# diffqc/dqc

Hardware: AMD Instinct MI355X
Metric: SCF iterations/sec (Fock build + XC grid) per GPU, cc-pVDZ 20-atom (higher is better)
Workload: dtype f64

## Files before the change

dqc_amd/csrc/grid_density.hip:

```cpp
#include "grid_common.hpp"

namespace dqc {

constexpr int DEN_BM = 64;
constexpr int DEN_NT = DEN_BM * 4;
constexpr int DEN_KC = 16;
constexpr int DEN_SA = DEN_KC + 2;

#ifdef DEN_TRACE
__device__ long long g_den_trace[4 * 16384];
DQC_DEV void den_trace(int k) {
    if (threadIdx.x == 0 && blockIdx.x < 16384) {
        if (k == 0) {
            unsigned hw, xcc;
            asm volatile("s_getreg_b32 %0, hwreg(HW_REG_HW_ID)" : "=s"(hw));
            asm volatile("s_getreg_b32 %0, hwreg(HW_REG_XCC_ID)" : "=s"(xcc));
            g_den_trace[4 * blockIdx.x + 3] = (long long)(((xcc & 7u) << 8) | ((hw >> 8) & 0xffu));
        }
        g_den_trace[4 * blockIdx.x + k] = wall_clock64();
    }
}
#define DEN_TRACE_POINT(k) den_trace(k)
#else
#define DEN_TRACE_POINT(k)
#endif

#ifdef DEN_EXP_UNPAIRED
constexpr bool DEN_PAIRED = false;
#else
constexpr bool DEN_PAIRED = true;
#endif

constexpr int lr_panel_stride(int nct) {
    return (DEN_PAIRED && nct >= 2) ? nct * 16 + 1 : (((nct * 16) & 31) == 16 ? nct * 16 : nct * 16 + 16);
}

template <int NCT, bool GGA, int Q0 = 0>
DQC_DEV void rowdot_epilogue(const v4d (&acc)[NCT], double (&p)[4][GGA ? 4 : 1], const double *__restrict__ blk0,
                             const double *__restrict__ blkg, size_t cs, const int (&roff)[4], int col0) {
    constexpr int NQ = (GGA ? 4 : 1) - Q0, NB = 4 * NQ;
    if (NB == 0) return;
    constexpr int DP = 2;
    double t[DP][NCT];
    auto issue = [&](int bt, double (&dst)[NCT]) {
        const int r = bt / NQ, q = bt % NQ + Q0;
        const double *base = (q == 0 ? blk0 : blkg + q * cs) + col0;
#pragma unroll
        for (int ct = 0; ct < NCT; ct++) dst[ct] = base[roff[r] + ct * 16];
    };
#pragma unroll
    for (int b0 = 0; b0 < DP - 1 && b0 < NB; b0++) issue(b0, t[b0]);
#pragma unroll
    for (int bt = 0; bt < NB; bt++) {
        if (bt + DP - 1 < NB) issue(bt + DP - 1, t[(bt + DP - 1) % DP]);
        const int r = bt / NQ, q = bt % NQ + Q0;
#pragma unroll
        for (int ct = 0; ct < NCT; ct++) p[r][q] += acc[ct][r] * t[bt % DP][ct];
        __builtin_amdgcn_sched_barrier(0);
    }
}

template <int NCT, bool GGA, int Q0 = 0, int DP = 2>
DQC_DEV void rowdot_epilogue_paired(const v4d (&acc)[NCT], double (&p)[4][GGA ? 4 : 1], const double *__restrict__ blk0,
                                    const double *__restrict__ blkg, size_t cs, const int (&roff)[4], int lr, int col0) {
    constexpr int NQ = (GGA ? 4 : 1) - Q0, NB = 4 * NQ, NP = NCT / 2, ODD = NCT & 1;
    if (NB == 0) return;
    double2 t2[DP][NP > 0 ? NP : 1];
    double t1[DP];
    auto issue = [&](int bt, double2 (&d2)[NP > 0 ? NP : 1], double &d1) {
        const int r = bt / NQ, q = bt % NQ + Q0;
        const double *base = (q == 0 ? blk0 : blkg + q * cs) + col0;
#pragma unroll
        for (int m = 0; m < NP; m++) d2[m] = *reinterpret_cast<const double2 *>(base + roff[r] + m * 32);
        if (ODD) d1 = base[(roff[r] - lr) + (NCT - 1) * 16];
    };
#pragma unroll
    for (int b0 = 0; b0 < DP - 1 && b0 < NB; b0++) issue(b0, t2[b0], t1[b0]);
#pragma unroll
    for (int bt = 0; bt < NB; bt++) {
        if (bt + DP - 1 < NB) issue(bt + DP - 1, t2[(bt + DP - 1) % DP], t1[(bt + DP - 1) % DP]);
        const int r = bt / NQ, q = bt % NQ + Q0;
#pragma unroll
        for (int m = 0; m < NP; m++) p[r][q] += acc[2 * m][r] * t2[bt % DP][m].x + acc[2 * m + 1][r] * t2[bt % DP][m].y;
        if (ODD) p[r][q] += acc[NCT - 1][r] * t1[bt % DP];
        __builtin_amdgcn_sched_barrier(0);
    }
}

template <int NCT>
DQC_DEV void rowdot_epilogue_paired2(const v4d (&acc)[2][NCT], double (&p)[2][4][4], const double *__restrict__ blkg, size_t cs,
                                     const int (&roff)[4], int lr, int col0) {
    constexpr int NQ = 3, NB = 4 * NQ, NP = NCT / 2, ODD = NCT & 1, DP = 2;
    double2 t2[DP][NP > 0 ? NP : 1];
    double t1[DP];
    auto issue = [&](int bt, double2 (&d2)[NP > 0 ? NP : 1], double &d1) {
        const int r = bt / NQ, q = bt % NQ + 1;
        const double *base = blkg + q * cs + col0;
#pragma unroll
        for (int m = 0; m < NP; m++) d2[m] = *reinterpret_cast<const double2 *>(base + roff[r] + m * 32);
        if (ODD) d1 = base[(roff[r] - lr) + (NCT - 1) * 16];
    };
    issue(0, t2[0], t1[0]);
#pragma unroll
    for (int bt = 0; bt < NB; bt++) {
        if (bt + 1 < NB) issue(bt + 1, t2[(bt + 1) % DP], t1[(bt + 1) % DP]);
        const int r = bt / NQ, q = bt % NQ + 1;
#pragma unroll
        for (int sp = 0; sp < 2; sp++) {
#pragma unroll
            for (int m = 0; m < NP; m++) p[sp][r][q] += acc[sp][2 * m][r] * t2[bt % DP][m].x + acc[sp][2 * m + 1][r] * t2[bt % DP][m].y;
            if (ODD) p[sp][r][q] += acc[sp][NCT - 1][r] * t1[bt % DP];
        }
        __builtin_amdgcn_sched_barrier(0);
    }
}

template <int NCT, bool GGA>
__global__ __launch_bounds__(256, 2) void density_kernel(double *__restrict__ rho, double *__restrict__ grho,
                                                         const double *__restrict__ ao, int ngrid, int ld,
                                                         const double *__restrict__ dm, int ntile,
                                                         const double *__restrict__ aoe, int lda) {
    extern __shared__ __attribute__((aligned(16))) double lds[];
    constexpr int LSB = NCT * 16;
    constexpr int LSBP = lr_panel_stride(NCT);
    constexpr int A_SZ = DEN_BM * DEN_SA, B_SZ = DEN_KC * LSBP;
    constexpr int NB2 = (DEN_KC * LSB / 2 + DEN_NT - 1) / DEN_NT;
    constexpr int NKK = DEN_KC / 4;
    double *sA = lds, *sB = lds + 2 * A_SZ;
    const int tid = threadIdx.x, wave = tid >> 6, lane = tid & 63;
    const int lr = lane & 15, lk = lane >> 4;
    const int g0 = blockIdx.x * DEN_BM;
    const size_t cs = (size_t)ngrid * lda;
    const double *aoblk = ao + (size_t)g0 * lda;
    const double *aoeblk = aoe + (size_t)g0 * lda;
    const int rmax = ngrid - 1 - g0;
    const int arow = tid >> 2, aseg = (tid & 3) * 4;
    const int aoff = min(arow, rmax) * lda + aseg;

    double p[4][GGA ? 4 : 1];
#pragma unroll
    for (int r = 0; r < 4; r++)
#pragma unroll
        for (int q = 0; q < (GGA ? 4 : 1); q++) p[r][q] = 0.0;
    int roff[4];
#pragma unroll
    for (int r = 0; r < 4; r++) roff[r] = min(wave * 16 + lk + 4 * r, rmax) * lda + (DEN_PAIRED ? 2 : 1) * lr;

    DEN_TRACE_POINT(0);
    const int nk = ld / DEN_KC;
    for (int jnew = 0; jnew < ntile; jnew += NCT) {
        const int jc = min(jnew, ntile - NCT);
        v4d acc[NCT];
#pragma unroll
        for (int ct = 0; ct < NCT; ct++) acc[ct] = v4d{0, 0, 0, 0};
        double2 paA0 = make_double2(0.0, 0.0), paA1 = paA0, paB0 = paA0, paB1 = paA0, pbA[NB2], pbB[NB2];
        int boff[NB2];
        bool bzero[NB2];
#pragma unroll
        for (int i = 0; i < NB2; i++) {
            const int e = min((tid + i * DEN_NT) * 2, DEN_KC * LSB - 2);
            const int row = e / LSB, col = e - row * LSB;
            boff[i] = row * ld + jc * 16 + col;
            bzero[i] = jc * 16 + col < jnew * 16;
            pbA[i] = pbB[i] = make_double2(0.0, 0.0);
        }
#define DQC_DEN_PREF(KC, S, PART)                                                                          \
    {                                                                                                      \
        const int kq_ = min((KC), nk - 1);      \
        if ((PART) == 0) {                                                                                 \
            const double *s_ = aoblk + kq_ * DEN_KC + aoff;                                                \
            pa##S##0 = *reinterpret_cast<const double2 *>(s_);                                             \
            pa##S##1 = *reinterpret_cast<const double2 *>(s_ + 2);                                         \
        }                                                                                                  \
        const double *d_ = dm + (size_t)kq_ * DEN_KC * ld;                                                 \
        _Pragma("unroll") for (int i = 0; i < NB2; i++) {                                                  \
            if (i % NKK != (PART)) continue;                                                               \
            pb##S[i] = *reinterpret_cast<const double2 *>(d_ + boff[i]);                                   \
            if (bzero[i]) pb##S[i] = make_double2(0.0, 0.0);                                               \
        }                                                                                                  \
    }
#define DQC_DEN_STAGE(KC, S)                                                                               \
    if ((KC) < nk) {                                                                                       \
        const int buf_ = (KC) & 1;                                                                         \
        double *a_ = sA + buf_ * A_SZ + arow * DEN_SA + aseg;                                              \
        *reinterpret_cast<double2 *>(a_) = pa##S##0;                                                       \
        *reinterpret_cast<double2 *>(a_ + 2) = pa##S##1;                                                   \
        _Pragma("unroll") for (int i = 0; i < NB2; i++) {                                                  \
            const int e = (tid + i * DEN_NT) * 2;                                                          \
            const int row = e / LSB, col = e - row * LSB;                                                  \
            if (row < DEN_KC) {                                     \
                double *d = sB + buf_ * B_SZ + row * LSBP + col;                                           \
                d[0] = pb##S[i].x;                                                                         \
                d[1] = pb##S[i].y;                                                                         \
            }                                                                                              \
        }                                                                                                  \
    }
#define DQC_DEN_MFMAS(KC, S)                                                                               \
    {                                                                                                      \
        const int buf_ = (KC) & 1;                                                                         \
        const double *a = sA + buf_ * A_SZ + (wave * 16 + lr) * DEN_SA + lk;                               \
        const double *b = sB + buf_ * B_SZ + lk * LSBP + lr;                                               \
        const double *b2 = b + lr;  \
        _Pragma("unroll") for (int kk = 0; kk < NKK; kk++) {                                               \
            DQC_DEN_PREF((KC) + 2, S, kk)                     \
            const double av = a[kk * 4];                                                                   \
            _Pragma("unroll") for (int ct = 0; ct < NCT; ct++) {                                           \
                const double bv = (DEN_PAIRED && ct < 2 * (NCT / 2)) ? b2[kk * 4 * LSBP + 32 * (ct >> 1) + (ct & 1)] \
                                                                    : b[kk * 4 * LSBP + ct * 16];          \
                acc[ct] = mfma_f64(av, bv, acc[ct]);                                                       \
            }                                                                                              \
        }                                                                                                  \
    }
        __syncthreads();
#pragma unroll
        for (int part = 0; part < NKK; part++) DQC_DEN_PREF(0, A, part)
#pragma unroll
        for (int part = 0; part < NKK; part++) DQC_DEN_PREF(1, B, part)
        DQC_DEN_STAGE(0, A)
        __syncthreads();
        int kc = 0;
        for (; kc + 1 < nk; kc += 2) {
            DQC_DEN_MFMAS(kc, A)
            DQC_DEN_STAGE(kc + 1, B)
            __syncthreads();
            DQC_DEN_MFMAS(kc + 1, B)
            DQC_DEN_STAGE(kc + 2, A)
            __syncthreads();
        }
        if (kc < nk) {
            DQC_DEN_MFMAS(kc, A)
            __syncthreads();
        }
#undef DQC_DEN_PREF
#undef DQC_DEN_STAGE
#undef DQC_DEN_MFMAS
        DEN_TRACE_POINT(1);
#ifdef ABL_DEN_NO_EPI
        if (ngrid < 0)
#endif
        {
            if constexpr (DEN_PAIRED) rowdot_epilogue_paired<NCT, GGA>(acc, p, GGA ? aoblk : aoeblk, aoblk, cs, roff, lr, jc * 16);
            else rowdot_epilogue<NCT, GGA>(acc, p, GGA ? aoblk : aoeblk, aoblk, cs, roff, jc * 16);
        }
    }
#pragma unroll
    for (int r = 0; r < 4; r++)
#pragma unroll
        for (int q = 0; q < (GGA ? 4 : 1); q++) {
            double v = p[r][q];
            v += __shfl_xor(v, 1);
            v += __shfl_xor(v, 2);
            v += __shfl_xor(v, 4);
            v += __shfl_xor(v, 8);
            p[r][q] = v;
        }
    DEN_TRACE_POINT(2);
    if (lr == 0) {
#pragma unroll
        for (int r = 0; r < 4; r++) {
            const int row = g0 + wave * 16 + lk + 4 * r;
            if (row < ngrid) {
                rho[row] = p[r][0];
                if (GGA) {
                    grho[row] = 2.0 * p[r][1];
                    grho[(size_t)ngrid + row] = 2.0 * p[r][2];
                    grho[2 * (size_t)ngrid + row] = 2.0 * p[r][3];
                }
            }
        }
    }
}

template <int NCT>
static constexpr size_t density_lds_bytes() {
    constexpr int LSBP = lr_panel_stride(NCT);
    return sizeof(double) * 2 * (DEN_BM * DEN_SA + DEN_KC * LSBP);
}

template <bool GGA>
static int launch_density(int nct, dim3 grid, hipStream_t st, double *rho, double *grho, const double *ao,
                          int ngrid, int ld, const double *dm, int ntile, const double *aoe, int lda) {

#define DQC_DENS_CASE(N)                                                                                           \
    case N:                                                                                                        \
        if constexpr (!GGA || N <= 14) {           \
            (void)hipFuncSetAttribute((const void *)density_kernel<N, GGA>, hipFuncAttributeMaxDynamicSharedMemorySize, \
                                      (int)density_lds_bytes<N>());                                                \
            hipLaunchKernelGGL((density_kernel<N, GGA>), grid, dim3(DEN_NT), density_lds_bytes<N>(), st, rho, grho, ao, \
                               ngrid, ld, dm, ntile, aoe, lda);                                                     \
            return 0;                                                                                              \
        }                                                                                                          \
        break;
    switch (nct) {
        DQC_DENS_CASE(1) DQC_DENS_CASE(2) DQC_DENS_CASE(3) DQC_DENS_CASE(4) DQC_DENS_CASE(5) DQC_DENS_CASE(6)
        DQC_DENS_CASE(7) DQC_DENS_CASE(8) DQC_DENS_CASE(9) DQC_DENS_CASE(10) DQC_DENS_CASE(11) DQC_DENS_CASE(12)
        DQC_DENS_CASE(13) DQC_DENS_CASE(14) DQC_DENS_CASE(15) DQC_DENS_CASE(16)
    default:
        break;
    }
#undef DQC_DENS_CASE
    set_error("density: internal tile-count dispatch error");
    return DQC_EINVAL;
}


template <int NRT>
struct LrGeom {
    static constexpr int RP = NRT * 16;
    static constexpr int RPS = (RP & 31) == 16 ? RP : RP + 16;
};

template <int NRT, int NCT, bool GGA, int NS = 1>
__global__ __launch_bounds__(256, 2) void density_lr_kernel(double *__restrict__ rho, double *__restrict__ grho,
                                                            const double *__restrict__ ao, int ngrid, int ld,
                                                            const double *__restrict__ orb,
                                                            const double *__restrict__ orbt, int ntile, int lda) {
    extern __shared__ __attribute__((aligned(16))) double lds[];
    constexpr int RP = LrGeom<NRT>::RP, RPS = LrGeom<NRT>::RPS;
    constexpr int LSB = NCT * 16;
    constexpr int LSBP = lr_panel_stride(NCT);
    constexpr int A_SZ = DEN_BM * DEN_SA;
    constexpr int B_SZ = DEN_KC * (LSBP > RPS ? LSBP : RPS);
    constexpr int NL2 = (DEN_KC * RP / 2 + DEN_NT - 1) / DEN_NT;
    constexpr int NB2 = (DEN_KC * LSB / 2 + DEN_NT - 1) / DEN_NT;
    double *sA = lds, *sB = lds + 2 * A_SZ;
    const int tid = threadIdx.x, wave = tid >> 6, lane = tid & 63;
    const int lr = lane & 15, lk = lane >> 4;
    const int g0 = blockIdx.x * DEN_BM;
    const size_t cs = (size_t)ngrid * lda;
    const double *aoblk = ao + (size_t)g0 * lda;
    const int rmax = ngrid - 1 - g0;
    const int arow = tid >> 2, aseg = (tid & 3) * 4;
    const int aoff = min(arow, rmax) * lda + aseg;

    DEN_TRACE_POINT(0);
    v4d a1[NRT];
#pragma unroll
    for (int ct = 0; ct < NRT; ct++) a1[ct] = v4d{0, 0, 0, 0};
    {
        static_assert(NL2 <= 4, "L chunk wider than 4 double2 per thread");
        double2 pa0a, pa0b, pa1a, pa1b, pl0a, pl0b, pl0c, pl0d, pl1a, pl1b, pl1c, pl1d;
        pl0a = pl0b = pl0c = pl0d = pl1a = pl1b = pl1c = pl1d = make_double2(0.0, 0.0);
        const int nk = ld / DEN_KC;
        const int lo0 = min((tid + 0 * DEN_NT) * 2, DEN_KC * RP - 2), lo1 = min((tid + 1 * DEN_NT) * 2, DEN_KC * RP - 2);
        const int lo2 = min((tid + 2 * DEN_NT) * 2, DEN_KC * RP - 2), lo3 = min((tid + 3 * DEN_NT) * 2, DEN_KC * RP - 2);
#define DQC_LR_PREFETCH(KC, S)                                                                            \
    {                                                                                                     \
        const int kq = min((KC), nk - 1);      \
        const double *s_ = aoblk + kq * DEN_KC + aoff;                                                    \
        pa##S##a = *reinterpret_cast<const double2 *>(s_);                                                \
        pa##S##b = *reinterpret_cast<const double2 *>(s_ + 2);                                            \
        const double *l_ = orb + (size_t)kq * DEN_KC * RP;  \
        pl##S##a = *reinterpret_cast<const double2 *>(l_ + lo0);                                          \
        if (NL2 > 1) pl##S##b = *reinterpret_cast<const double2 *>(l_ + lo1);                             \
        if (NL2 > 2) pl##S##c = *reinterpret_cast<const double2 *>(l_ + lo2);                             \
        if (NL2 > 3) pl##S##d = *reinterpret_cast<const double2 *>(l_ + lo3);                             \
    }
#define DQC_LR_PUT(I, V)                                                                                  \
    {                                                                                                     \
        const int e_ = (tid + (I) * DEN_NT) * 2;                                                          \
        const int row_ = e_ / RP, col_ = e_ - row_ * RP;                                                  \
        if (row_ < DEN_KC) *reinterpret_cast<double2 *>(sB + buf_ * B_SZ + row_ * RPS + col_) = V;        \
    }
#define DQC_LR_STAGE(KC, S)                                                                               \
    if ((KC) < nk) {                                                                                      \
        const int buf_ = (KC) & 1;                                                                        \
        double *a_ = sA + buf_ * A_SZ + arow * DEN_SA + aseg;                                             \
        *reinterpret_cast<double2 *>(a_) = pa##S##a;                                                      \
        *reinterpret_cast<double2 *>(a_ + 2) = pa##S##b;                                                  \
        DQC_LR_PUT(0, pl##S##a)                                                                           \
        if (NL2 > 1) DQC_LR_PUT(1, pl##S##b)                                                              \
        if (NL2 > 2) DQC_LR_PUT(2, pl##S##c)                                                              \
        if (NL2 > 3) DQC_LR_PUT(3, pl##S##d)                                                              \
    }
#define DQC_LR_MFMAS(KC)                                                                                  \
    {                                                                                                     \
        const int buf_ = (KC) & 1;                                                                        \
        const double *b_ = sA + buf_ * A_SZ + (wave * 16 + lr) * DEN_SA + lk;  \
        const double *a_ = sB + buf_ * B_SZ + lk * RPS + lr;                   \
        _Pragma("unroll") for (int kk = 0; kk < DEN_KC / 4; kk++) {                                       \
            const double bv = b_[kk * 4];                                                                 \
            _Pragma("unroll") for (int ct = 0; ct < NRT; ct++)                                            \
                a1[ct] = mfma_f64(a_[kk * 4 * RPS + ct * 16], bv, a1[ct]);                                \
        }                                                                                                 \
    }
        DQC_LR_PREFETCH(0, 0)
        DQC_LR_PREFETCH(1, 1)
        DQC_LR_STAGE(0, 0)
        __syncthreads();
        int kc = 0;
        for (; kc + 1 < nk; kc += 2) {
            DQC_LR_PREFETCH(kc + 2, 0)
            DQC_LR_MFMAS(kc)
            DQC_LR_STAGE(kc + 1, 1)
            __syncthreads();
            DQC_LR_PREFETCH(kc + 3, 1)
            DQC_LR_MFMAS(kc + 1)
            DQC_LR_STAGE(kc + 2, 0)
            __syncthreads();
        }
        if (kc < nk) {
            DQC_LR_MFMAS(kc)
            __syncthreads();
        }
#undef DQC_LR_PREFETCH
#undef DQC_LR_STAGE
#undef DQC_LR_PUT
#undef DQC_LR_MFMAS
    }

    static_assert(NS == 1 || (NS == 2 && NRT % 2 == 0), "two spin channels of equal padded width");
    constexpr int NRU = NRT / NS;
#pragma unroll
    for (int sp = 0; sp < NS; sp++) {
        double rs = 0.0;
#pragma unroll
        for (int ct = sp * NRU; ct < (sp + 1) * NRU; ct++)
#pragma unroll
            for (int q = 0; q < 4; q++) rs += a1[ct][q] * a1[ct][q];
        rs += __shfl_xor(rs, 16);
        rs += __shfl_xor(rs, 32);
        const int row = g0 + wave * 16 + lr;
        if (lk == 0 && row < ngrid) rho[(size_t)sp * ngrid + row] = rs;
    }
    if (!GGA) return;

    double p[NS][4][GGA ? 4 : 1];
#pragma unroll
    for (int sp = 0; sp < NS; sp++)
#pragma unroll
    for (int r = 0; r < 4; r++)
#pragma unroll
        for (int q = 0; q < (GGA ? 4 : 1); q++) p[sp][r][q] = 0.0;
    int roff[4];
#pragma unroll
    for (int r = 0; r < 4; r++) roff[r] = min(wave * 16 + lk + 4 * r, rmax) * lda + (DEN_PAIRED ? 2 : 1) * lr;

    for (int jnew = 0; jnew < ntile; jnew += NCT) {
        const int jc = min(jnew, ntile - NCT);
        v4d acc[NS][NCT];
#pragma unroll
        for (int sp = 0; sp < NS; sp++)
#pragma unroll
        for (int ct = 0; ct < NCT; ct++) acc[sp][ct] = v4d{0, 0, 0, 0};
        double2 pb[NB2];
        int boff[NB2];
        bool bzero[NB2];
#pragma unroll
        for (int i = 0; i < NB2; i++) {
            const int e = min((tid + i * DEN_NT) * 2, DEN_KC * LSB - 2);
            const int row = e / LSB, col = e - row * LSB;
            boff[i] = row * ld + jc * 16 + col;
            bzero[i] = jc * 16 + col < jnew * 16;
        }
        auto prefetch = [&](int kc) {
            const double *l = orbt + (size_t)kc * DEN_KC * ld;
#pragma unroll
            for (int i = 0; i < NB2; i++) {
                pb[i] = *reinterpret_cast<const double2 *>(l + boff[i]);
                if (bzero[i]) pb[i] = make_double2(0.0, 0.0);
            }
        };
        auto stage = [&](int buf) {
#pragma unroll
            for (int i = 0; i < NB2; i++) {
                const int e = (tid + i * DEN_NT) * 2;
                const int row = e / LSB, col = e - row * LSB;
                if (row < DEN_KC) {
                    double *d = sB + buf * B_SZ + row * LSBP + col;
                    d[0] = pb[i].x;
                    d[1] = pb[i].y;
                }
            }
        };
        __syncthreads();
        prefetch(0);
        stage(0);
        __syncthreads();
#pragma unroll 1
        for (int kc = 0; kc < NRT; kc++) {
            const int buf = kc & 1;
            if (kc + 1 < NRT) prefetch(kc + 1);
            v4d a4 = a1[0];
#pragma unroll
            for (int c = 1; c < NRT; c++)
                if (kc == c) a4 = a1[c];
            const double *b = sB + buf * B_SZ + lk * LSBP + lr;
            const double *b2 = b + lr;
#pragma unroll
            for (int kk = 0; kk < 4; kk++) {
                const double av = a4[kk];
#pragma unroll
                for (int ct = 0; ct < NCT; ct++) {
                    const double bv = (DEN_PAIRED && ct < 2 * (NCT / 2)) ? b2[kk * 4 * LSBP + 32 * (ct >> 1) + (ct & 1)]
                                                                        : b[kk * 4 * LSBP + ct * 16];
                    if (NS == 1 || kc < NRU) acc[0][ct] = mfma_f64(av, bv, acc[0][ct]);
                    else acc[NS - 1][ct] = mfma_f64(av, bv, acc[NS - 1][ct]);
                }
            }
            if (kc + 1 < NRT) stage(buf ^ 1);
            __syncthreads();
        }
        DEN_TRACE_POINT(1);
        if constexpr (NS == 2) {
            static_assert(NS == 1 || (DEN_PAIRED && GGA), "spin-fused form: paired epilogue only");
            rowdot_epilogue_paired2<NCT>(acc, p, aoblk, cs, roff, lr, jc * 16);
        } else if constexpr (!DEN_PAIRED) rowdot_epilogue<NCT, GGA, 1>(acc[0], p[0], aoblk, aoblk, cs, roff, jc * 16);
        else if constexpr (GGA) rowdot_epilogue_paired<NCT, true, 1>(acc[0], p[0], aoblk, aoblk, cs, roff, lr, jc * 16);
        DEN_TRACE_POINT(2);
    }
#pragma unroll
    for (int sp = 0; sp < NS; sp++)
#pragma unroll
    for (int r = 0; r < 4; r++)
#pragma unroll
        for (int q = 0; q < (GGA ? 4 : 1); q++) {
            double v = p[sp][r][q];
            v += __shfl_xor(v, 1);
            v += __shfl_xor(v, 2);
            v += __shfl_xor(v, 4);
            v += __shfl_xor(v, 8);
            p[sp][r][q] = v;
        }
    if (lr == 0) {
#pragma unroll
        for (int sp = 0; sp < NS; sp++)
#pragma unroll
        for (int r = 0; r < 4; r++) {
            const int row = g0 + wave * 16 + lk + 4 * r;
            if (row < ngrid) {
                double *gs = grho + (size_t)sp * 3 * ngrid;
                gs[row] = 2.0 * p[sp][r][1];
                gs[(size_t)ngrid + row] = 2.0 * p[sp][r][2];
                gs[2 * (size_t)ngrid + row] = 2.0 * p[sp][r][3];
            }
        }
    }
}

template <int NRT, int NCT>
static constexpr size_t density_lr_lds_bytes() {
    constexpr int LSBP = lr_panel_stride(NCT);
    constexpr int RPS = LrGeom<NRT>::RPS;
    return sizeof(double) * 2 * (DEN_BM * DEN_SA + DEN_KC * (LSBP > RPS ? LSBP : RPS));
}

constexpr int lr_max_nct(int nrt) { return nrt <= 3 ? 14 : (nrt <= 4 ? 12 : 10); }

template <int NRT, bool GGA>
static int launch_density_lr_n(int nct, dim3 grid, hipStream_t st, double *rho, double *grho, const double *ao, int ngrid,
                               int ld, const double *orb, const double *orbt, int ntile, int lda) {
#define DQC_DLR_CASE(N)                                                                                          \
    case N:                                                                                                      \
        if constexpr (!GGA || N <= lr_max_nct(NRT)) {          \
            constexpr size_t shm = density_lr_lds_bytes<NRT, N>();                                               \
            auto kern = density_lr_kernel<NRT, N, GGA>;                                                          \
            (void)hipFuncSetAttribute((const void *)kern, hipFuncAttributeMaxDynamicSharedMemorySize, (int)shm); \
            hipLaunchKernelGGL(kern, grid, dim3(DEN_NT), shm, st, rho, grho, ao, ngrid, ld, orb, orbt, ntile, lda); \
            return 0;                                                                                            \
        }                                                                                                        \
        break;
    switch (nct) {
        DQC_DLR_CASE(1) DQC_DLR_CASE(2) DQC_DLR_CASE(3) DQC_DLR_CASE(4) DQC_DLR_CASE(5) DQC_DLR_CASE(6) DQC_DLR_CASE(7)
        DQC_DLR_CASE(8) DQC_DLR_CASE(9) DQC_DLR_CASE(10) DQC_DLR_CASE(11) DQC_DLR_CASE(12) DQC_DLR_CASE(13) DQC_DLR_CASE(14)
        DQC_DLR_CASE(15) DQC_DLR_CASE(16)
    default:
        break;
    }
#undef DQC_DLR_CASE
    set_error("density_lr: internal tile-count dispatch error");
    return DQC_EINVAL;
}

constexpr int ROLE_NT = 512;
constexpr unsigned ROLE_SPIN_CAP = 1u << 22;
constexpr int ROLE_DP = 3;

template <int NRT, int NT>
struct RoleGeom {
    static constexpr int RP = NRT * 16;
    static constexpr int S = NT * 16 + 1;
    static constexpr int P0 = (NT + 1) / 2;
    static constexpr int P1 = NT - P0;
    static constexpr int LT_SZ = (RP * S + 1) & ~1;
    static constexpr int MB_W = P0 * 256;
    static constexpr int SA_W = 2 * 16 * DEN_SA;
    static constexpr size_t lds_bytes() { return sizeof(double) * (LT_SZ + 4 * MB_W + 4 * SA_W) + 64; }
};

template <int NT>
DQC_DEV int role_col(int ct, int lr) {
    return ct < 2 * (NT / 2) ? 32 * (ct >> 1) + 2 * lr + (ct & 1) : ct * 16 + lr;
}

DQC_DEV void role_wait(unsigned *flag, unsigned want, unsigned *broken) {
    unsigned n = 0;
    while (__hip_atomic_load(flag, __ATOMIC_ACQUIRE, __HIP_MEMORY_SCOPE_WORKGROUP) < want) {
        if (__hip_atomic_load(broken, __ATOMIC_RELAXED, __HIP_MEMORY_SCOPE_WORKGROUP) != 0u) break;
        if (++n > ROLE_SPIN_CAP) {
            __hip_atomic_store(broken, 1u, __ATOMIC_RELAXED, __HIP_MEMORY_SCOPE_WORKGROUP);
            break;
        }
        __builtin_amdgcn_s_sleep(2);
    }
}

DQC_DEV void role_signal(unsigned *flag, unsigned v) {
    __hip_atomic_store(flag, v, __ATOMIC_RELEASE, __HIP_MEMORY_SCOPE_WORKGROUP);
}

template <int NRT, int NT>
__global__ __launch_bounds__(ROLE_NT, 1) void density_roles_kernel(double *__restrict__ rho, double *__restrict__ grho,
                                                                   const double *__restrict__ ao, int ngrid,
                                                                   const double *__restrict__ orbt, int lda) {
    using G = RoleGeom<NRT, NT>;
    constexpr int RP = G::RP, S = G::S, P0 = G::P0, P1 = G::P1, LD = NT * 16;
    constexpr int NPF = 4;
    static_assert(NT >= 2 && NT <= 14 && P1 >= 1, "one epilogue panel of 2..14 tiles");
    extern __shared__ __attribute__((aligned(16))) double lds[];
    double *sLT = lds, *sMB = lds + G::LT_SZ, *sAall = sMB + 4 * G::MB_W;
    unsigned *flags = reinterpret_cast<unsigned *>(sAall + 4 * G::SA_W);
    const int tid = threadIdx.x, lane = tid & 63;
    const int wave = __builtin_amdgcn_readfirstlane(tid >> 6);
    const int lr = lane & 15, lk = lane >> 4;
    const int ntiles = (ngrid + DEN_BM - 1) / DEN_BM;
    const size_t cs = (size_t)ngrid * lda;

    for (int e = tid; e < RP * LD; e += ROLE_NT) {
        const int r = e / LD, c = e - r * LD;
        sLT[r * S + c] = orbt[e];
    }
    if (tid < 16) flags[tid] = 0u;
    __syncthreads();
    const int w = wave & 3;
    unsigned *filled = flags + w, *drained = flags + 4 + w, *broken = flags + 8;
    double *mb = sMB + w * G::MB_W + lane * 2;
    unsigned seq = 0;

    if (wave < 4) {
        double *sA = sAall + w * G::SA_W;
        const int arow = lane >> 2, aseg = (lane & 3) * 4;
        double2 pa0a, pa0b, pa1a, pa1b, pa2a, pa2b, pa3a, pa3b;
        static_assert(NPF == 4, "four named prefetch sets");
#define DQC_ROLE_REQUEST(T, KC, SET)                                                                       \
    {                                                         \
        const int rmax_ = ngrid - 1 - (T) * DEN_BM;                                                        \
        const double *s_ = ao + (size_t)(T) * DEN_BM * lda + (min(w * 16 + arow, rmax_) * lda + aseg) + (KC) * DEN_KC; \
        pa##SET##a = *reinterpret_cast<const double2 *>(s_);                                               \
        pa##SET##b = *reinterpret_cast<const double2 *>(s_ + 2);                                           \
    }
#define DQC_ROLE_STEP(KC, SET)                                                                             \
    if ((KC) < NT) {                                                                                       \
        double *a_ = sA + ((KC) & 1) * 16 * DEN_SA;                                                        \
        *reinterpret_cast<double2 *>(a_ + arow * DEN_SA + aseg) = pa##SET##a;                              \
        *reinterpret_cast<double2 *>(a_ + arow * DEN_SA + aseg + 2) = pa##SET##b;                          \
        if ((KC) + NPF < NT) DQC_ROLE_REQUEST(t, (KC) + NPF, SET)                                          \
        __builtin_amdgcn_fence(__ATOMIC_RELEASE, "wavefront");                                             \
        __builtin_amdgcn_wave_barrier();  \
        __builtin_amdgcn_fence(__ATOMIC_ACQUIRE, "wavefront");                                             \
        const double *b_ = a_ + lr * DEN_SA + lk;                            \
        const double *l_ = sLT + lr * S + (KC) * DEN_KC + lk;                \
        _Pragma("unroll") for (int kk = 0; kk < DEN_KC / 4; kk++) {                                        \
            const double bv = b_[kk * 4];                                                                  \
            _Pragma("unroll") for (int ct = 0; ct < NRT; ct++)                                             \
                a1[ct] = mfma_f64(l_[ct * 16 * S + kk * 4], bv, a1[ct]);                                   \
        }                                                                                                  \
    }
#define DQC_ROLE_REQUEST4(T)  \
    DQC_ROLE_REQUEST(T, 0, 0) DQC_ROLE_REQUEST(T, 1, 1) DQC_ROLE_REQUEST(T, 2, 2) DQC_ROLE_REQUEST(T, 3, 3)
        int t = blockIdx.x;
        pa0a = pa0b = pa1a = pa1b = pa2a = pa2b = pa3a = pa3b = make_double2(0.0, 0.0);
        if (t < ntiles) { DQC_ROLE_REQUEST4(t) }
        for (; t < ntiles; t += gridDim.x) {
            const int g0 = t * DEN_BM;
            v4d a1[NRT];
#pragma unroll
            for (int ct = 0; ct < NRT; ct++) a1[ct] = v4d{0, 0, 0, 0};
            DQC_ROLE_STEP(0, 0) DQC_ROLE_STEP(1, 1) DQC_ROLE_STEP(2, 2) DQC_ROLE_STEP(3, 3) DQC_ROLE_STEP(4, 0)
            DQC_ROLE_STEP(5, 1) DQC_ROLE_STEP(6, 2) DQC_ROLE_STEP(7, 3) DQC_ROLE_STEP(8, 0) DQC_ROLE_STEP(9, 1)
            DQC_ROLE_STEP(10, 2) DQC_ROLE_STEP(11, 3) DQC_ROLE_STEP(12, 0) DQC_ROLE_STEP(13, 1)
            {
                double rs = 0.0;
#pragma unroll
                for (int ct = 0; ct < NRT; ct++)
#pragma unroll
                    for (int q = 0; q < 4; q++) rs += a1[ct][q] * a1[ct][q];
                rs += __shfl_xor(rs, 16);
                rs += __shfl_xor(rs, 32);
                const int row = g0 + w * 16 + lr;
                if (lk == 0 && row < ngrid) rho[row] = rs;
            }
            if (t + (int)gridDim.x < ntiles) { DQC_ROLE_REQUEST4(t + (int)gridDim.x) }
#pragma unroll
            for (int h = 0; h < 2; h++) {
                constexpr int PMAX = P0;
                const int c0 = h * P0;
                v4d acc[PMAX];
#pragma unroll
                for (int ct = 0; ct < PMAX; ct++) acc[ct] = v4d{0, 0, 0, 0};
#pragma unroll
                for (int kc = 0; kc < NRT; kc++)
#pragma unroll
                    for (int kk = 0; kk < 4; kk++) {
                        const double av = a1[kc][kk];
                        const double *b = sLT + (kc * 16 + kk * 4 + lk) * S;
#pragma unroll
                        for (int ct = 0; ct < PMAX; ct++)
                            if (ct < (h ? P1 : P0)) acc[ct] = mfma_f64(av, b[role_col<NT>(c0 + ct, lr)], acc[ct]);
                    }
                role_wait(drained, seq, broken);
#pragma unroll
                for (int ct = 0; ct < PMAX; ct++)
                    if (ct < (h ? P1 : P0)) {
                        *reinterpret_cast<double2 *>(mb + (2 * ct) * 128) = make_double2(acc[ct][0], acc[ct][1]);
                        *reinterpret_cast<double2 *>(mb + (2 * ct + 1) * 128) = make_double2(acc[ct][2], acc[ct][3]);
                    }
                seq++;
                role_signal(filled, seq);
            }
        }
#undef DQC_ROLE_REQUEST4
#undef DQC_ROLE_STEP
#undef DQC_ROLE_REQUEST
    } else {
        for (int t = blockIdx.x; t < ntiles; t += gridDim.x) {
            const int g0 = t * DEN_BM;
            const int rmax = ngrid - 1 - g0;
            const double *aoblk = ao + (size_t)g0 * lda;
            int roff[4];
#pragma unroll
            for (int r = 0; r < 4; r++) roff[r] = min(w * 16 + lk + 4 * r, rmax) * lda + 2 * lr;
            v4d acc[NT];
#pragma unroll
            for (int h = 0; h < 2; h++) {
                role_wait(filled, seq + 1, broken);
#pragma unroll
                for (int ct = 0; ct < (h ? P1 : P0); ct++) {
                    const double2 lo = *reinterpret_cast<const double2 *>(mb + (2 * ct) * 128);
                    const double2 hi = *reinterpret_cast<const double2 *>(mb + (2 * ct + 1) * 128);
                    acc[h * P0 + ct] = v4d{lo.x, lo.y, hi.x, hi.y};
                }
                seq++;
                role_signal(drained, seq);
            }
            double p[4][4];
#pragma unroll
            for (int r = 0; r < 4; r++)
#pragma unroll
                for (int q = 0; q < 4; q++) p[r][q] = 0.0;
            rowdot_epilogue_paired<NT, true, 1, ROLE_DP>(acc, p, aoblk, aoblk, cs, roff, lr, 0);
#pragma unroll
            for (int r = 0; r < 4; r++)
#pragma unroll
                for (int q = 1; q < 4; q++) {
                    double v = p[r][q];
                    v += __shfl_xor(v, 1);
                    v += __shfl_xor(v, 2);
                    v += __shfl_xor(v, 4);
                    v += __shfl_xor(v, 8);
                    p[r][q] = v;
                }
            const bool bad = __hip_atomic_load(broken, __ATOMIC_RELAXED, __HIP_MEMORY_SCOPE_WORKGROUP) != 0u;
            if (lr == 0) {
#pragma unroll
                for (int r = 0; r < 4; r++) {
                    const int row = g0 + w * 16 + lk + 4 * r;
                    if (row < ngrid) {
                        const double nan = __builtin_nan("");
                        grho[row] = bad ? nan : 2.0 * p[r][1];
                        grho[(size_t)ngrid + row] = bad ? nan : 2.0 * p[r][2];
                        grho[2 * (size_t)ngrid + row] = bad ? nan : 2.0 * p[r][3];
                    }
                }
            }
        }
    }
}

static bool density_roles_shape(int nrt, int ntile) { return nrt == 3 && ntile == 13; }

static bool density_roles_enabled() {
    const char *e = getenv("DQC_DENSITY_ROLES");
    return !(e && e[0] == '0');
}

static int launch_density_roles(int nrt, int ntile, hipStream_t st, double *rho, double *grho, const double *ao, int ngrid,
                                const double *orbt, int lda) {
    static int ncu = 0;
    if (ncu == 0) {
        int dev = 0, n = 0;
        if (hipGetDevice(&dev) != hipSuccess || hipDeviceGetAttribute(&n, hipDeviceAttributeMultiprocessorCount, dev) != hipSuccess || n <= 0) {
            set_error("density_roles: cannot read the device's CU count");
            return DQC_EINVAL;
        }
        ncu = n;
    }
    const int ntiles = (ngrid + DEN_BM - 1) / DEN_BM;
    if (nrt == 3 && ntile == 13) {
        constexpr size_t shm = RoleGeom<3, 13>::lds_bytes();
        static_assert(shm <= 160 * 1024, "one block has to fit the CU's LDS");
        auto kern = density_roles_kernel<3, 13>;
        (void)hipFuncSetAttribute((const void *)kern, hipFuncAttributeMaxDynamicSharedMemorySize, (int)shm);
        hipLaunchKernelGGL(kern, dim3(std::min(ntiles, ncu)), dim3(ROLE_NT), shm, st, rho, grho, ao, ngrid, orbt, lda);
        return 0;
    }
    set_error("density_roles: internal shape dispatch error");
    return DQC_EINVAL;
}

template <int NRT>
__global__ __launch_bounds__(256, 2) void density_lr_tau_kernel(double *__restrict__ rho, double *__restrict__ grho, double *__restrict__ tau,
                                                                const double *__restrict__ ao, int ngrid, int ld,
                                                                const double *__restrict__ orb, int lda) {
    extern __shared__ __attribute__((aligned(16))) double lds[];
    constexpr int RP = LrGeom<NRT>::RP, RPS = LrGeom<NRT>::RPS;
    constexpr int A_SZ = DEN_BM * DEN_SA, B_SZ = DEN_KC * RPS;
    constexpr int NL2 = (DEN_KC * RP / 2 + DEN_NT - 1) / DEN_NT;
    static_assert(NL2 <= 4, "L chunk wider than 4 double2 per thread");
    double *sA = lds, *sB = lds + 4 * A_SZ;
    const int tid = threadIdx.x, wave = tid >> 6, lane = tid & 63;
    const int lr = lane & 15, lk = lane >> 4;
    const int g0 = blockIdx.x * DEN_BM;
    const size_t cs = (size_t)ngrid * lda;
    const double *aoblk = ao + (size_t)g0 * lda;
    const int rmax = ngrid - 1 - g0;
    const int arow = tid >> 2, aseg = (tid & 3) * 4;
    const int aoff = min(arow, rmax) * lda + aseg;
    const int nk = ld / DEN_KC;
    const int lo0 = min((tid + 0 * DEN_NT) * 2, DEN_KC * RP - 2), lo1 = min((tid + 1 * DEN_NT) * 2, DEN_KC * RP - 2);
    const int lo2 = min((tid + 2 * DEN_NT) * 2, DEN_KC * RP - 2), lo3 = min((tid + 3 * DEN_NT) * 2, DEN_KC * RP - 2);

    v4d psi[NRT];
    double rs = 0.0, ts = 0.0, gs[3] = {0.0, 0.0, 0.0};
#pragma unroll 1
    for (int pair = 0; pair < 2; pair++) {
        const double *blk0 = aoblk + (size_t)(2 * pair) * cs, *blk1 = blk0 + cs;
        v4d a0[NRT], a1[NRT];
#pragma unroll
        for (int ct = 0; ct < NRT; ct++) a0[ct] = a1[ct] = v4d{0, 0, 0, 0};
        double2 x0a, x0b, y0a, y0b, x1a, x1b, y1a, y1b, pl0a, pl0b, pl0c, pl0d, pl1a, pl1b, pl1c, pl1d;
        pl0a = pl0b = pl0c = pl0d = pl1a = pl1b = pl1c = pl1d = make_double2(0.0, 0.0);
#define DQC_LT_PREFETCH(KC, S)                                                                            \
    {                                                                                                     \
        const int kq = min((KC), nk - 1);      \
        const double *s0_ = blk0 + kq * DEN_KC + aoff, *s1_ = blk1 + kq * DEN_KC + aoff;                  \
        x##S##a = *reinterpret_cast<const double2 *>(s0_);                                                \
        x##S##b = *reinterpret_cast<const double2 *>(s0_ + 2);                                            \
        y##S##a = *reinterpret_cast<const double2 *>(s1_);                                                \
        y##S##b = *reinterpret_cast<const double2 *>(s1_ + 2);                                            \
        const double *l_ = orb + (size_t)kq * DEN_KC * RP;                                                \
        pl##S##a = *reinterpret_cast<const double2 *>(l_ + lo0);                                          \
        if (NL2 > 1) pl##S##b = *reinterpret_cast<const double2 *>(l_ + lo1);                             \
        if (NL2 > 2) pl##S##c = *reinterpret_cast<const double2 *>(l_ + lo2);                             \
        if (NL2 > 3) pl##S##d = *reinterpret_cast<const double2 *>(l_ + lo3);                             \
    }
#define DQC_LT_PUT(I, V)                                                                                  \
    {                                                                                                     \
        const int e_ = (tid + (I) * DEN_NT) * 2;                                                          \
        const int row_ = e_ / RP, col_ = e_ - row_ * RP;                                                  \
        if (row_ < DEN_KC) *reinterpret_cast<double2 *>(sB + buf_ * B_SZ + row_ * RPS + col_) = V;        \
    }
#define DQC_LT_STAGE(KC, S)                                                                               \
    if ((KC) < nk) {                                                                                      \
        const int buf_ = (KC) & 1;                                                                        \
        double *a_ = sA + buf_ * 2 * A_SZ + arow * DEN_SA + aseg;                                         \
        *reinterpret_cast<double2 *>(a_) = x##S##a;                                                       \
        *reinterpret_cast<double2 *>(a_ + 2) = x##S##b;                                                   \
        *reinterpret_cast<double2 *>(a_ + A_SZ) = y##S##a;                                                \
        *reinterpret_cast<double2 *>(a_ + A_SZ + 2) = y##S##b;                                            \
        DQC_LT_PUT(0, pl##S##a)                                                                           \
        if (NL2 > 1) DQC_LT_PUT(1, pl##S##b)                                                              \
        if (NL2 > 2) DQC_LT_PUT(2, pl##S##c)                                                              \
        if (NL2 > 3) DQC_LT_PUT(3, pl##S##d)                                                              \
    }
#define DQC_LT_MFMAS(KC)                                                                                  \
    {                                                                                                     \
        const int buf_ = (KC) & 1;                                                                        \
        const double *b_ = sA + buf_ * 2 * A_SZ + (wave * 16 + lr) * DEN_SA + lk;  \
        const double *l_ = sB + buf_ * B_SZ + lk * RPS + lr;                       \
        _Pragma("unroll") for (int kk = 0; kk < DEN_KC / 4; kk++) {                                       \
            const double bv0 = b_[kk * 4], bv1 = b_[A_SZ + kk * 4];                                       \
            _Pragma("unroll") for (int ct = 0; ct < NRT; ct++) {                                          \
                const double lv = l_[kk * 4 * RPS + ct * 16];                                             \
                a0[ct] = mfma_f64(lv, bv0, a0[ct]);                                                       \
                a1[ct] = mfma_f64(lv, bv1, a1[ct]);                                                       \
            }                                                                                             \
        }                                                                                                 \
    }
        __syncthreads();
        DQC_LT_PREFETCH(0, 0)
        DQC_LT_PREFETCH(1, 1)
        DQC_LT_STAGE(0, 0)
        __syncthreads();
        int kc = 0;
        for (; kc + 1 < nk; kc += 2) {
            DQC_LT_PREFETCH(kc + 2, 0)
            DQC_LT_MFMAS(kc)
            DQC_LT_STAGE(kc + 1, 1)
            __syncthreads();
            DQC_LT_PREFETCH(kc + 3, 1)
            DQC_LT_MFMAS(kc + 1)
            DQC_LT_STAGE(kc + 2, 0)
            __syncthreads();
        }
        if (kc < nk) {
            DQC_LT_MFMAS(kc)
            __syncthreads();
        }
#undef DQC_LT_PREFETCH
#undef DQC_LT_STAGE
#undef DQC_LT_PUT
#undef DQC_LT_MFMAS
        if (pair == 0) {
#pragma unroll
            for (int ct = 0; ct < NRT; ct++) {
                psi[ct] = a0[ct];
#pragma unroll
                for (int q = 0; q < 4; q++) {
                    rs += a0[ct][q] * a0[ct][q];
                    gs[0] += a0[ct][q] * a1[ct][q];
                    ts += a1[ct][q] * a1[ct][q];
                }
            }
        } else {
#pragma unroll
            for (int ct = 0; ct < NRT; ct++)
#pragma unroll
                for (int q = 0; q < 4; q++) {
                    gs[1] += psi[ct][q] * a0[ct][q];
                    gs[2] += psi[ct][q] * a1[ct][q];
                    ts += a0[ct][q] * a0[ct][q] + a1[ct][q] * a1[ct][q];
                }
        }
    }
    double out[5] = {rs, 2.0 * gs[0], 2.0 * gs[1], 2.0 * gs[2], 0.5 * ts};
#pragma unroll
    for (int q = 0; q < 5; q++) {
        out[q] += __shfl_xor(out[q], 16);
        out[q] += __shfl_xor(out[q], 32);
    }
    const int row = g0 + wave * 16 + lr;
    if (lk == 0 && row < ngrid) {
        rho[row] = out[0];
        grho[row] = out[1];
        grho[(size_t)ngrid + row] = out[2];
        grho[2 * (size_t)ngrid + row] = out[3];
        tau[row] = out[4];
    }
}

constexpr int lr2_max_nct(int nrt) { return nrt <= 4 ? 6 : (nrt <= 6 ? 5 : 4); }

template <int NRT>
static int launch_density_lr2_n(int nct, dim3 grid, hipStream_t st, double *rho, double *grho, const double *ao, int ngrid, int ld,
                                const double *orb, const double *orbt, int ntile, int lda) {
#define DQC_DLR2_CASE(N)                                                                                         \
    case N:                                                                                                      \
        if constexpr (N <= lr2_max_nct(NRT)) {                                                                   \
            constexpr size_t shm = density_lr_lds_bytes<NRT, N>();                                               \
            auto kern = density_lr_kernel<NRT, N, true, 2>;                                                      \
            (void)hipFuncSetAttribute((const void *)kern, hipFuncAttributeMaxDynamicSharedMemorySize, (int)shm); \
            hipLaunchKernelGGL(kern, grid, dim3(DEN_NT), shm, st, rho, grho, ao, ngrid, ld, orb, orbt, ntile, lda); \
            return 0;                                                                                            \
        }                                                                                                        \
        break;
    switch (nct) {
        DQC_DLR2_CASE(1) DQC_DLR2_CASE(2) DQC_DLR2_CASE(3) DQC_DLR2_CASE(4) DQC_DLR2_CASE(5) DQC_DLR2_CASE(6) DQC_DLR2_CASE(7)
    default:
        break;
    }
#undef DQC_DLR2_CASE
    set_error("density_lr (two spins): internal tile-count dispatch error");
    return DQC_EINVAL;
}

template <bool GGA>
static int launch_density_lr(int nrt, int nct, dim3 grid, hipStream_t st, double *rho, double *grho, const double *ao,
                             int ngrid, int ld, const double *orb, const double *orbt, int ntile, int lda) {
    switch (nrt) {
    case 1: return launch_density_lr_n<1, GGA>(nct, grid, st, rho, grho, ao, ngrid, ld, orb, orbt, ntile, lda);
    case 2: return launch_density_lr_n<2, GGA>(nct, grid, st, rho, grho, ao, ngrid, ld, orb, orbt, ntile, lda);
    case 3: return launch_density_lr_n<3, GGA>(nct, grid, st, rho, grho, ao, ngrid, ld, orb, orbt, ntile, lda);
    case 4: return launch_density_lr_n<4, GGA>(nct, grid, st, rho, grho, ao, ngrid, ld, orb, orbt, ntile, lda);
    case 6: return launch_density_lr_n<6, GGA>(nct, grid, st, rho, grho, ao, ngrid, ld, orb, orbt, ntile, lda);
    case 8: return launch_density_lr_n<8, GGA>(nct, grid, st, rho, grho, ao, ngrid, ld, orb, orbt, ntile, lda);
    default:
        set_error("density_lr: internal factor-width dispatch error");
        return DQC_EINVAL;
    }
}

}

extern "C" {

int dqc_grid_density(double *d_rho, double *d_grho, const double *d_ao, int ncomp, int ngrid, int nao,
                     const double *d_dm, void *stream) {
    using namespace dqc;
    hipStream_t st = (hipStream_t)stream;
    if (ngrid <= 0) return DQC_OK;
    const bool gga = d_grho != nullptr;
    if (gga && ncomp < 4) { set_error("dqc_grid_density: gradient requested but ao has < 4 components"); return DQC_EINVAL; }
    const int ld = dqc_padded_nao(nao), ntile = ld / 16, lda = dqc_ao_stride(nao);
    const int nchunk = (ntile + (gga ? 13 : 15)) / (gga ? 14 : 16);
    const int nct = (ntile + nchunk - 1) / nchunk;
    dim3 grid((ngrid + DEN_BM - 1) / DEN_BM);
    int rc = gga ? launch_density<true>(nct, grid, st, d_rho, d_grho, d_ao, ngrid, ld, d_dm, ntile, d_ao, lda)
                 : launch_density<false>(nct, grid, st, d_rho, d_grho, d_ao, ngrid, ld, d_dm, ntile, d_ao, lda);
    if (rc) return rc;
    DQC_CHECK_LAUNCH();
    return DQC_OK;
}

int dqc_padded_norb(int norb) {
    static const int sizes[] = {16, 32, 48, 64, 96, 128};
    for (int sz : sizes)
        if (norb <= sz) return sz;
    return 0;
}

int dqc_grid_density_lr(double *d_rho, double *d_grho, const double *d_ao, int ncomp, int ngrid, int nao,
                        const double *d_orb, const double *d_orbt, int norb_pad, void *stream) {
    using namespace dqc;
    hipStream_t st = (hipStream_t)stream;
    if (ngrid <= 0) return DQC_OK;
    const bool gga = d_grho != nullptr;
    if (gga && ncomp < 4) { set_error("dqc_grid_density_lr: gradient requested but ao has < 4 components"); return DQC_EINVAL; }
    if (norb_pad <= 0 || dqc_padded_norb(norb_pad) != norb_pad) {
        set_error("dqc_grid_density_lr: norb_pad must be a value returned by dqc_padded_norb");
        return DQC_EINVAL;
    }
    const int ld = dqc_padded_nao(nao), ntile = ld / 16, lda = dqc_ao_stride(nao);
    const int lim = gga ? dqc::lr_max_nct(norb_pad / 16) : 16;
    const int nchunk = (ntile + lim - 1) / lim;
    const int nct = (ntile + nchunk - 1) / nchunk;
    dim3 grid((ngrid + DEN_BM - 1) / DEN_BM);
    int rc;
    if (gga && density_roles_shape(norb_pad / 16, ntile) && density_roles_enabled())
        rc = launch_density_roles(norb_pad / 16, ntile, st, d_rho, d_grho, d_ao, ngrid, d_orbt, lda);
    else
        rc = gga ? launch_density_lr<true>(norb_pad / 16, nct, grid, st, d_rho, d_grho, d_ao, ngrid, ld, d_orb, d_orbt, ntile, lda)
                 : launch_density_lr<false>(norb_pad / 16, nct, grid, st, d_rho, d_grho, d_ao, ngrid, ld, d_orb, d_orbt, ntile, lda);
    if (rc) return rc;
    DQC_CHECK_LAUNCH();
    return DQC_OK;
}

int dqc_grid_density_lr_roles(int nao, int norb_pad, int gga) {
    using namespace dqc;
    if (!gga || norb_pad <= 0 || dqc_padded_norb(norb_pad) != norb_pad) return 0;
    return density_roles_shape(norb_pad / 16, dqc_padded_nao(nao) / 16) && density_roles_enabled() ? 1 : 0;
}

int dqc_grid_density_lr_pol(double *d_rho, double *d_grho, const double *d_ao, int ncomp, int ngrid, int nao,
                            const double *d_orb, const double *d_orbt, int norb_pad_spin, void *stream) {
    using namespace dqc;
    hipStream_t st = (hipStream_t)stream;
    if (ngrid <= 0) return DQC_OK;
    if (!d_grho || ncomp < 4) { set_error("dqc_grid_density_lr_pol: needs the four AO components and the gradient output"); return DQC_EINVAL; }
    if (norb_pad_spin != 16 && norb_pad_spin != 32 && norb_pad_spin != 48 && norb_pad_spin != 64) {
        set_error("dqc_grid_density_lr_pol: norb_pad_spin must be 16, 32, 48 or 64");
        return DQC_EINVAL;
    }
    const int ld = dqc_padded_nao(nao), ntile = ld / 16, lda = dqc_ao_stride(nao);
    const int nrt = 2 * norb_pad_spin / 16;
    const int lim = lr2_max_nct(nrt);
    const int nchunk = (ntile + lim - 1) / lim;
    const int nct = (ntile + nchunk - 1) / nchunk;
    dim3 grid((ngrid + DEN_BM - 1) / DEN_BM);
    int rc;
    switch (nrt) {
    case 2: rc = launch_density_lr2_n<2>(nct, grid, st, d_rho, d_grho, d_ao, ngrid, ld, d_orb, d_orbt, ntile, lda); break;
    case 4: rc = launch_density_lr2_n<4>(nct, grid, st, d_rho, d_grho, d_ao, ngrid, ld, d_orb, d_orbt, ntile, lda); break;
    case 6: rc = launch_density_lr2_n<6>(nct, grid, st, d_rho, d_grho, d_ao, ngrid, ld, d_orb, d_orbt, ntile, lda); break;
    default: rc = launch_density_lr2_n<8>(nct, grid, st, d_rho, d_grho, d_ao, ngrid, ld, d_orb, d_orbt, ntile, lda); break;
    }
    if (rc) return rc;
    DQC_CHECK_LAUNCH();
    return DQC_OK;
}

int dqc_grid_density_pair(double *d_out, const double *d_ao_a, const double *d_ao_b, int ngrid, int nao,
                          const double *d_dm, void *stream) {
    using namespace dqc;
    hipStream_t st = (hipStream_t)stream;
    if (ngrid <= 0) return DQC_OK;
    const int ld = dqc_padded_nao(nao), ntile = ld / 16, lda = dqc_ao_stride(nao);
    const int nchunk = (ntile + 15) / 16;
    const int nct = (ntile + nchunk - 1) / nchunk;
    dim3 grid((ngrid + DEN_BM - 1) / DEN_BM);
    int rc = launch_density<false>(nct, grid, st, d_out, nullptr, d_ao_a, ngrid, ld, d_dm, ntile, d_ao_b, lda);
    if (rc) return rc;
    DQC_CHECK_LAUNCH();
    return DQC_OK;
}

int dqc_grid_density_lr_tau(double *d_rho, double *d_grho, double *d_tau, const double *d_ao, int ncomp, int ngrid, int nao,
                            const double *d_orb, int norb_pad, void *stream) {
    using namespace dqc;
    hipStream_t st = (hipStream_t)stream;
    if (ngrid <= 0) return DQC_OK;
    if (ncomp < 4 || !d_grho || !d_tau) { set_error("dqc_grid_density_lr_tau: needs the four AO components and all three outputs"); return DQC_EINVAL; }
    if (norb_pad <= 0 || dqc_padded_norb(norb_pad) != norb_pad) {
        set_error("dqc_grid_density_lr_tau: norb_pad must be a value returned by dqc_padded_norb");
        return DQC_EINVAL;
    }
    const int ld = dqc_padded_nao(nao), lda = dqc_ao_stride(nao);
    dim3 grid((ngrid + DEN_BM - 1) / DEN_BM);
#define DQC_LT_CASE(N)                                                                                                         \
    case N: {                                                                                                                  \
        constexpr size_t bytes = sizeof(double) * (4 * DEN_BM * DEN_SA + 2 * DEN_KC * LrGeom<N>::RPS);                         \
        (void)hipFuncSetAttribute((const void *)density_lr_tau_kernel<N>, hipFuncAttributeMaxDynamicSharedMemorySize, (int)bytes); \
        hipLaunchKernelGGL((density_lr_tau_kernel<N>), grid, dim3(DEN_NT), bytes, st, d_rho, d_grho, d_tau, d_ao, ngrid, ld, d_orb, lda); \
    } break;
    switch (norb_pad / 16) {
        DQC_LT_CASE(1) DQC_LT_CASE(2) DQC_LT_CASE(3) DQC_LT_CASE(4) DQC_LT_CASE(6)
    default:
        set_error("dqc_grid_density_lr_tau: factors wider than 96 columns are not supported");
        return DQC_EINVAL;
    }
#undef DQC_LT_CASE
    DQC_CHECK_LAUNCH();
    return DQC_OK;
}

}
```

Before: 797.9.

## Prefetch next tile's AO epilogue loads across tiles in density roles kernel

Adds a cross-tile software pipeline to the epilogue waves of the role-split density kernel. The first batches of AO row loads for the next tile are issued during the tail of the current tile's rowdot, and the loop is peeled so the last tile issues no lookahead. This aims to hide global-load latency at tile boundaries, where each tile's epilogue used to restart its prefetch from cold. It keeps more double2 registers live across the loop and the role handshake, and adds a compile-time PIPE variant chosen by an environment variable that is on by default.

```diff
diff --git a/dqc_amd/csrc/grid_density.hip b/dqc_amd/csrc/grid_density.hip
--- a/dqc_amd/csrc/grid_density.hip
+++ b/dqc_amd/csrc/grid_density.hip
@@ -1,3 +1,5 @@
+#include <type_traits>
+
 #include "grid_common.hpp"
 
 namespace dqc {
@@ -83,6 +85,44 @@
 #pragma unroll
         for (int m = 0; m < NP; m++) p[r][q] += acc[2 * m][r] * t2[bt % DP][m].x + acc[2 * m + 1][r] * t2[bt % DP][m].y;
         if (ODD) p[r][q] += acc[NCT - 1][r] * t1[bt % DP];
+        __builtin_amdgcn_sched_barrier(0);
+    }
+}
+
+template <int NCT, bool GGA, int Q0>
+DQC_DEV void rowdot_paired_issue(int bt, double2 (&d2)[NCT / 2 > 0 ? NCT / 2 : 1], double &d1, const double *__restrict__ blk0,
+                                 const double *__restrict__ blkg, size_t cs, const int (&roff)[4], int lr, int col0) {
+    constexpr int NQ = (GGA ? 4 : 1) - Q0, NP = NCT / 2, ODD = NCT & 1;
+    const int r = bt / NQ, q = bt % NQ + Q0;
+    const double *base = (q == 0 ? blk0 : blkg + q * cs) + col0;
+#pragma unroll
+    for (int m = 0; m < NP; m++) d2[m] = *reinterpret_cast<const double2 *>(base + roff[r] + m * 32);
+    if (ODD) d1 = base[(roff[r] - lr) + (NCT - 1) * 16];
+}
+
+template <int NCT, bool GGA, int Q0, int DP, bool AHEAD>
+DQC_DEV void rowdot_paired_xt(const v4d (&acc)[NCT], double (&p)[4][GGA ? 4 : 1], const double *__restrict__ blk0,
+                              const double *__restrict__ blkg, size_t cs, const int (&roff)[4], int lr, int col0,
+                              double2 (&t2)[DP][NCT / 2 > 0 ? NCT / 2 : 1], double (&t1)[DP], const double *__restrict__ nblk0,
+                              const double *__restrict__ nblkg, const int (&nroff)[4]) {
+    constexpr int NQ = (GGA ? 4 : 1) - Q0, NB = 4 * NQ, NP = NCT / 2, ODD = NCT & 1;
+    static_assert(NB % DP == 0 && NB >= 2 * DP, "batch b of every panel lands in register set b % DP");
+#pragma unroll
+    for (int bt = 0; bt < NB; bt++) {
+        const int nb = bt + DP - 1;
+        if (nb >= NB) {
+            if constexpr (AHEAD) rowdot_paired_issue<NCT, GGA, Q0>(nb - NB, t2[nb % DP], t1[nb % DP], nblk0, nblkg, cs, nroff, lr, col0);
+        } else if (bt >= 1) {
+            rowdot_paired_issue<NCT, GGA, Q0>(nb, t2[nb % DP], t1[nb % DP], blk0, blkg, cs, roff, lr, col0);
+        }
+        const int r = bt / NQ, q = bt % NQ + Q0;
+#pragma unroll
+        for (int m = 0; m < NP; m++) p[r][q] += acc[2 * m][r] * t2[bt % DP][m].x + acc[2 * m + 1][r] * t2[bt % DP][m].y;
+        if (ODD) p[r][q] += acc[NCT - 1][r] * t1[bt % DP];
+        __builtin_amdgcn_sched_barrier(0);
+    }
+    if constexpr (AHEAD) {
+        rowdot_paired_issue<NCT, GGA, Q0>(DP - 1, t2[DP - 1], t1[DP - 1], nblk0, nblkg, cs, nroff, lr, col0);
         __builtin_amdgcn_sched_barrier(0);
     }
 }
@@ -609,7 +649,7 @@
     __hip_atomic_store(flag, v, __ATOMIC_RELEASE, __HIP_MEMORY_SCOPE_WORKGROUP);
 }
 
-template <int NRT, int NT>
+template <int NRT, int NT, bool PIPE>
 __global__ __launch_bounds__(ROLE_NT, 1) void density_roles_kernel(double *__restrict__ rho, double *__restrict__ grho,
                                                                    const double *__restrict__ ao, int ngrid,
                                                                    const double *__restrict__ orbt, int lda) {
@@ -723,7 +763,16 @@
 #undef DQC_ROLE_STEP
 #undef DQC_ROLE_REQUEST
     } else {
-        for (int t = blockIdx.x; t < ntiles; t += gridDim.x) {
+        constexpr int NPB = NT / 2 > 0 ? NT / 2 : 1;
+        double2 t2[ROLE_DP][NPB];
+        double t1[ROLE_DP];
+        auto tile_roff = [&](int tt, int (&ro)[4]) {
+            const int rmax = ngrid - 1 - tt * DEN_BM;
+#pragma unroll
+            for (int r = 0; r < 4; r++) ro[r] = min(w * 16 + lk + 4 * r, rmax) * lda + 2 * lr;
+        };
+        auto tile = [&](int t, auto ahead) {
+            constexpr bool AHEAD = decltype(ahead)::value;
             const int g0 = t * DEN_BM;
             const int rmax = ngrid - 1 - g0;
             const double *aoblk = ao + (size_t)g0 * lda;
@@ -743,12 +792,17 @@
                 seq++;
                 role_signal(drained, seq);
             }
+            __builtin_amdgcn_sched_barrier(0);
             double p[4][4];
 #pragma unroll
             for (int r = 0; r < 4; r++)
 #pragma unroll
                 for (int q = 0; q < 4; q++) p[r][q] = 0.0;
-            rowdot_epilogue_paired<NT, true, 1, ROLE_DP>(acc, p, aoblk, aoblk, cs, roff, lr, 0);
+            const int tn = AHEAD ? t + (int)gridDim.x : t;
+            int nroff[4];
+            tile_roff(tn, nroff);
+            const double *nblk = ao + (size_t)tn * DEN_BM * lda;
+            rowdot_paired_xt<NT, true, 1, ROLE_DP, AHEAD>(acc, p, aoblk, aoblk, cs, roff, lr, 0, t2, t1, nblk, nblk, nroff);
 #pragma unroll
             for (int r = 0; r < 4; r++)
 #pragma unroll
@@ -773,6 +827,73 @@
                     }
                 }
             }
+        };
+        if constexpr (PIPE) {
+            int t = blockIdx.x;
+            if (t < ntiles) {
+                int roff0[4];
+                tile_roff(t, roff0);
+                const double *blk = ao + (size_t)t * DEN_BM * lda;
+#pragma unroll
+                for (int b0 = 0; b0 < ROLE_DP; b0++) {
+                    rowdot_paired_issue<NT, true, 1>(b0, t2[b0], t1[b0], blk, blk, cs, roff0, lr, 0);
+                    __builtin_amdgcn_sched_barrier(0);
+                }
+                for (; t + (int)gridDim.x < ntiles; t += gridDim.x) tile(t, std::true_type{});
+                tile(t, std::false_type{});
+            }
+        } else {
+            for (int t = blockIdx.x; t < ntiles; t += gridDim.x) {
+                const int g0 = t * DEN_BM;
+                const int rmax = ngrid - 1 - g0;
+                const double *aoblk = ao + (size_t)g0 * lda;
+                int roff[4];
+    #pragma unroll
+                for (int r = 0; r < 4; r++) roff[r] = min(w * 16 + lk + 4 * r, rmax) * lda + 2 * lr;
+                v4d acc[NT];
+    #pragma unroll
+                for (int h = 0; h < 2; h++) {
+                    role_wait(filled, seq + 1, broken);
+    #pragma unroll
+                    for (int ct = 0; ct < (h ? P1 : P0); ct++) {
+                        const double2 lo = *reinterpret_cast<const double2 *>(mb + (2 * ct) * 128);
+                        const double2 hi = *reinterpret_cast<const double2 *>(mb + (2 * ct + 1) * 128);
+                        acc[h * P0 + ct] = v4d{lo.x, lo.y, hi.x, hi.y};
+                    }
+                    seq++;
+                    role_signal(drained, seq);
+                }
+                double p[4][4];
+    #pragma unroll
+                for (int r = 0; r < 4; r++)
+    #pragma unroll
+                    for (int q = 0; q < 4; q++) p[r][q] = 0.0;
+                rowdot_epilogue_paired<NT, true, 1, ROLE_DP>(acc, p, aoblk, aoblk, cs, roff, lr, 0);
+    #pragma unroll
+                for (int r = 0; r < 4; r++)
+    #pragma unroll
+                    for (int q = 1; q < 4; q++) {
+                        double v = p[r][q];
+                        v += __shfl_xor(v, 1);
+                        v += __shfl_xor(v, 2);
+                        v += __shfl_xor(v, 4);
+                        v += __shfl_xor(v, 8);
+                        p[r][q] = v;
+                    }
+                const bool bad = __hip_atomic_load(broken, __ATOMIC_RELAXED, __HIP_MEMORY_SCOPE_WORKGROUP) != 0u;
+                if (lr == 0) {
+    #pragma unroll
+                    for (int r = 0; r < 4; r++) {
+                        const int row = g0 + w * 16 + lk + 4 * r;
+                        if (row < ngrid) {
+                            const double nan = __builtin_nan("");
+                            grho[row] = bad ? nan : 2.0 * p[r][1];
+                            grho[(size_t)ngrid + row] = bad ? nan : 2.0 * p[r][2];
+                            grho[2 * (size_t)ngrid + row] = bad ? nan : 2.0 * p[r][3];
+                        }
+                    }
+                }
+            }
         }
     }
 }
@@ -781,6 +902,11 @@
 
 static bool density_roles_enabled() {
     const char *e = getenv("DQC_DENSITY_ROLES");
+    return !(e && e[0] == '0');
+}
+
+static bool density_roles_pipe_enabled() {
+    const char *e = getenv("DQC_DENSITY_ROLES_PIPE");
     return !(e && e[0] == '0');
 }
 
@@ -799,7 +925,7 @@
     if (nrt == 3 && ntile == 13) {
         constexpr size_t shm = RoleGeom<3, 13>::lds_bytes();
         static_assert(shm <= 160 * 1024, "one block has to fit the CU's LDS");
-        auto kern = density_roles_kernel<3, 13>;
+        auto kern = density_roles_pipe_enabled() ? density_roles_kernel<3, 13, true> : density_roles_kernel<3, 13, false>;
         (void)hipFuncSetAttribute((const void *)kern, hipFuncAttributeMaxDynamicSharedMemorySize, (int)shm);
         hipLaunchKernelGGL(kern, dim3(std::min(ntiles, ncu)), dim3(ROLE_NT), shm, st, rho, grho, ao, ngrid, orbt, lda);
         return 0;
```

Result: no change. 797.3 (-0.1%).
